# Onetism/LightFieldMicroscopy_PC-bzip2

Measured on AMD Instinct MI355X. Metric: uint16 Mpixel/s encode (predictor->bzip2) at 1/2/4/8 GPUs; ratio parity, higher is better.
Workload: dtype u16

## Files before the change

lightfieldmicroscopy_pc-bzip2_amd/csrc/lfm_bzip2.hip:

```cpp
#include <hip/hip_runtime.h>
#include <rocprim/block/block_exchange.hpp>
#include <rocprim/block/block_sort.hpp>
#include <rocprim/device/device_radix_sort.hpp>
#include <rocprim/device/device_scan.hpp>
#include <rocprim/device/device_segmented_radix_sort.hpp>
#include <rocprim/device/device_select.hpp>
#include <rocprim/iterator/counting_iterator.hpp>
#include <algorithm>
#include <climits>
#include <cstdlib>
#include <cstdint>
#include <cstdio>
#include <cstring>
#include <mutex>
#include <type_traits>
#include <vector>
#include "lfm_bwt_types.h"
#include "lfm_bz_caps.h"
#include "lfm_hip.h"

#ifndef LFM_BWT_FORCE_FULL
#define LFM_BWT_FORCE_FULL 0
#endif

namespace lfm {
namespace bz {

constexpr int kRleThreads = 512;
constexpr int kMaxGroups = 6;
constexpr int kMaxAlpha = 258;
constexpr int kIters = 4;
constexpr uint32_t kRunA = 0, kRunB = 1;

constexpr uint32_t kFlagHost = 1;

struct Geometry {
    uint32_t dims[5];
    uint32_t bs[5];
    uint32_t nb[5];
    uint32_t bpp;
};

struct Batch {
    const uint8_t* img;
    Geometry g;
    uint32_t first_block;
    uint32_t nstreams;
    uint32_t raw_cap;
    uint32_t cap;
    uint32_t level;
    uint32_t nblock_max;
    uint32_t out_cap;
    uint8_t* raw;
    uint32_t* raw_len;
    uint8_t* T;
    uint32_t* n;
    uint32_t* crc;
    uint32_t* inuse;
    uint32_t* flags;
    uint32_t* done;
    uint64_t* keys_a;
    uint64_t* keys_b;
    uint32_t* vals_a;
    uint32_t* sa;
    uint32_t* rank;
    uint32_t* vals_b;
    uint32_t* cl0;
    uint32_t* cl1;
    uint8_t* uflag;
    uint32_t* seg_begin;
    uint32_t* seg_end;
    uint16_t* mtfv;
    uint32_t* nmtf;
    uint32_t* mtf_freq;
    uint32_t* orig_ptr;
    uint8_t* sel;
    uint8_t* sel_mtf;
    uint32_t sel_cap;
    uint32_t* nsel;
    uint32_t* ngroups;
    uint8_t* len;
    uint32_t* code;
    uint32_t* rfreq;
    uint32_t* words;
    uint32_t* out_bytes;
    uint32_t* wide;
    uint32_t* wide_cnt;
    uint32_t* nsub;
    uint32_t* bwt_mode;
    uint32_t* abcnt;
    uint32_t* itab;
    uint2* ent;
    uint32_t it_full;
    uint32_t parts;
    uint32_t full_cap;
    uint8_t* Tfull;
    uint32_t* part_toff;
    uint32_t* part_roff;
    uint32_t* part_rlen;
    uint32_t* out_bits;
    uint32_t* nparts;
    uint32_t* sflags;
    uint32_t* sbytes;
    uint32_t* jwords;
    uint32_t jcap;
    uint32_t pay_cap;
};

__device__ __forceinline__ void block_box(const Geometry& g, uint32_t id, uint32_t org[5], uint32_t sz[5])
{
#pragma unroll
    for (int d = 0; d < 5; ++d) {
        const uint32_t q = id % g.nb[d];
        id /= g.nb[d];
        org[d] = q * g.bs[d];
        sz[d] = min(g.bs[d], g.dims[d] - org[d]);
    }
}

__global__ __launch_bounds__(256) void gather_blocks(Batch B)
{
    const uint32_t s = blockIdx.y;
    uint32_t org[5], sz[5];
    block_box(B.g, B.first_block + s, org, sz);
    const uint32_t rowb = sz[0] * B.g.bpp;
    const uint32_t nrows = sz[1] * sz[2] * sz[3] * sz[4];
    uint8_t* dst = B.raw + (size_t)s * B.raw_cap;
    for (uint32_t r = blockIdx.x; r < nrows; r += gridDim.x) {
        uint32_t q = r;
        const uint32_t y = q % sz[1]; q /= sz[1];
        const uint32_t z = q % sz[2]; q /= sz[2];
        const uint32_t c = q % sz[3]; q /= sz[3];
        const uint32_t t = q;
        const size_t src = ((((size_t)(org[4] + t) * B.g.dims[3] + (org[3] + c)) * B.g.dims[2] + (org[2] + z)) *
                                B.g.dims[1] + (org[1] + y)) * B.g.dims[0] + org[0];
        const uint8_t* sp = B.img + src * B.g.bpp;
        uint8_t* dp = dst + (size_t)r * rowb;
        for (uint32_t i = threadIdx.x; i < rowb; i += blockDim.x) dp[i] = sp[i];
    }
    if (blockIdx.x == 0 && threadIdx.x == 0) B.raw_len[s] = rowb * nrows;
}

struct RunSum {
    uint32_t len;
    uint32_t first, last;
    uint32_t lead;
    uint32_t trail;
};

__device__ __forceinline__ RunSum run_combine(const RunSum& a, const RunSum& b)
{
    const bool ae = a.len == 0, be = b.len == 0;
    const bool join = a.last == b.first && !ae && !be;
    RunSum r;
    r.len = a.len + b.len;
    r.first = ae ? b.first : a.first;
    r.last = be ? a.last : b.last;
    r.lead = ae ? b.lead : ((join && a.lead == a.len) ? a.len + b.lead : a.lead);
    r.trail = be ? a.trail : ((join && b.trail == b.len) ? b.len + a.trail : b.trail);
    return r;
}

__device__ __forceinline__ RunSum run_shfl_up(const RunSum& a, int d)
{
    RunSum r;
    r.len = __shfl_up(a.len, d);
    r.first = __shfl_up(a.first, d);
    r.last = __shfl_up(a.last, d);
    r.lead = __shfl_up(a.lead, d);
    r.trail = __shfl_up(a.trail, d);
    return r;
}
// ... 2236 lines not shown
            tile_out[rle2_swz(wr + w - 1u)] = (uint16_t)EOB;
            atomicAdd(&freq[EOB], 1u);
        }
        __syncthreads();
        const uint32_t base = s_wr;
        for (uint32_t i = t; i < tile_total; i += kRle2Threads) out[base + i] = tile_out[rle2_swz(i)];
        __syncthreads();
        if (t == 0) {
            s_wr = base + tile_total;
            s_carry = tile_end_zeros;
        }
        __syncthreads();
    }
    static_assert(kRunA == 0 && kRunB == 1, "RUNA / RUNB are symbols 0 and 1");
    uint32_t cnts[6] = {nrunA, nrunB, (uint32_t)(hot & 0xFFFFu), (uint32_t)((hot >> 16) & 0xFFFFu),
                        (uint32_t)((hot >> 32) & 0xFFFFu), (uint32_t)(hot >> 48)};
#pragma unroll
    for (int r = 0; r < 6; ++r) {
        uint32_t c = cnts[r];
        for (int d = 32; d > 0; d >>= 1) c += (uint32_t)__shfl_xor((int)c, d);
        if (lane == 0 && c) atomicAdd(&freq[r], c);
    }
    __syncthreads();
    if (t == 0) {
        B.nmtf[s] = s_wr;
        if (!heap_narrow(B, s, (int)nin + 2)) B.wide[atomicAdd(B.wide_cnt, 1u)] = s;
    }
    for (uint32_t v = t; v < kMaxAlpha; v += kRle2Threads) B.mtf_freq[(size_t)s * kMaxAlpha + v] = freq[v];
}

constexpr int kHuffThreads = 256;

__device__ __forceinline__ uint32_t stream_nin(const Batch& B, uint32_t s)
{
    uint32_t nin = 0;
    for (int q = 0; q < 8; ++q) nin += __popc(B.inuse[s * 8 + q]);
    return nin;
}

__global__ __launch_bounds__(64) void huff_init(Batch B)
{
    __shared__ int mf[kMaxAlpha];
    __shared__ int pgs[kMaxGroups], pge[kMaxGroups];
    const uint32_t s = blockIdx.x, t = threadIdx.x;
    if (B.flags[s] & kFlagHost) return;
    const uint32_t nMTF = B.nmtf[s];
    const int alphaSize = (int)stream_nin(B, s) + 2;
    const uint32_t* mfreq = B.mtf_freq + (size_t)s * kMaxAlpha;
    uint8_t* len = B.len + (size_t)s * kMaxGroups * kMaxAlpha;
    const int nGroups = nMTF < 200 ? 2 : nMTF < 600 ? 3 : nMTF < 1200 ? 4 : nMTF < 2400 ? 5 : 6;
    for (int v = t; v < kMaxAlpha; v += 64) mf[v] = v < alphaSize ? (int)mfreq[v] : 0;
    __syncthreads();
    if (t == 0) {
        int nPart = nGroups, remF = (int)nMTF, gs = 0;
        while (nPart > 0) {
            const int tFreq = remF / nPart;
            int ge = gs - 1, aFreq = 0;
            while (aFreq < tFreq && ge < alphaSize - 1) {
                ++ge;
                aFreq += mf[ge];
            }
            if (ge > gs && nPart != nGroups && nPart != 1 && ((nGroups - nPart) % 2 == 1)) {
                aFreq -= mf[ge];
                --ge;
            }
            pgs[nPart - 1] = gs;
            pge[nPart - 1] = ge;
            --nPart;
            gs = ge + 1;
            remF -= aFreq;
        }
        B.ngroups[s] = (uint32_t)nGroups;
        B.nsel[s] = (nMTF + kGSize - 1) / kGSize;
    }
    __syncthreads();
    for (int i = t; i < kMaxGroups * kMaxAlpha; i += 64) {
        const int q = i / kMaxAlpha, v = i - q * kMaxAlpha;
        len[i] = (q < nGroups && v < alphaSize && v >= pgs[q] && v <= pge[q]) ? 0 : 15;
    }
}

__global__ __launch_bounds__(kHuffThreads) void huff_select_reg(Batch B)
{
    __shared__ uint32_t rfreq[kMaxGroups][kMaxAlpha];
    __shared__ uint64_t lpack[kMaxAlpha + 1];
    __shared__ uint32_t junk[kHuffThreads];
    const uint32_t s = blockIdx.x, t = threadIdx.x;
    if (B.flags[s] & kFlagHost) return;
    const uint32_t nMTF = B.nmtf[s], nSel = B.nsel[s];
    const int nGroups = (int)B.ngroups[s];
    const int alphaSize = (int)stream_nin(B, s) + 2;
    const uint8_t* len = B.len + (size_t)s * kMaxGroups * kMaxAlpha;
    const uint16_t* mtfv = B.mtfv + (size_t)s * (B.cap + 8);
    uint8_t* sel = B.sel + (size_t)s * B.sel_cap;
    for (int i = t; i < kMaxGroups * kMaxAlpha; i += kHuffThreads) rfreq[i / kMaxAlpha][i % kMaxAlpha] = 0;
    for (int v = t; v <= kMaxAlpha; v += kHuffThreads) {
        uint64_t lp = 0;
        if (v < alphaSize)
            for (int q = 0; q < nGroups; ++q) lp |= (uint64_t)len[q * kMaxAlpha + v] << (10 * q);
        lpack[v] = lp;
    }
    __syncthreads();
    uint64_t lp_hot[4];
#pragma unroll
    for (int f = 0; f < 4; ++f) lp_hot[f] = lpack[f];
    for (uint32_t g = t; g < nSel; g += kHuffThreads) {
        const uint32_t gs = g * kGSize, cnt = min(nMTF - gs, (uint32_t)kGSize);
        uint32_t w[kGSize / 2];
        if (cnt == (uint32_t)kGSize) {
            const uint32_t* p = (const uint32_t*)(mtfv + gs);
#pragma unroll
            for (int q = 0; q < kGSize / 2; ++q) w[q] = p[q];
        } else {
#pragma unroll
            for (int q = 0; q < kGSize / 2; ++q) {
                const uint32_t lo = 2u * q < cnt ? mtfv[gs + 2 * q] : (uint32_t)kMaxAlpha;
                const uint32_t hi = 2u * q + 1 < cnt ? mtfv[gs + 2 * q + 1] : (uint32_t)kMaxAlpha;
                w[q] = lo | (hi << 16);
            }
        }
        uint32_t hot = 0;
        uint64_t acc = 0;
#pragma unroll
        for (int q = 0; q < kGSize / 2; ++q) {
            const uint32_t lo = w[q] & 0xFFFFu, hi = w[q] >> 16;
            hot += lo < 4u ? 1u << (8u * lo) : 0u;
            hot += hi < 4u ? 1u << (8u * hi) : 0u;
            acc += lpack[lo < 4u ? (uint32_t)kMaxAlpha : lo] + lpack[hi < 4u ? (uint32_t)kMaxAlpha : hi];
        }
#pragma unroll
        for (uint32_t f = 0; f < 4; ++f) acc += (uint64_t)((hot >> (8u * f)) & 0xFFu) * lp_hot[f];
        int bt = -1;
        uint32_t bc = 999999999u;
        for (int q = 0; q < nGroups; ++q) {
            const uint32_t cq = (uint32_t)(acc >> (10 * q)) & 1023u;
            if (cq < bc) { bc = cq; bt = q; }
        }
        sel[g] = (uint8_t)bt;
#pragma unroll
        for (int q = 0; q < kGSize / 2; ++q) {
            const uint32_t lo = w[q] & 0xFFFFu, hi = w[q] >> 16;
            atomicAdd(lo >= 4u && lo != (uint32_t)kMaxAlpha ? &rfreq[bt][lo] : &junk[t], 1u);
            atomicAdd(hi >= 4u && hi != (uint32_t)kMaxAlpha ? &rfreq[bt][hi] : &junk[t], 1u);
        }
#pragma unroll
        for (uint32_t f = 0; f < 4; ++f)
            if ((hot >> (8u * f)) & 0xFFu) atomicAdd(&rfreq[bt][f], (hot >> (8u * f)) & 0xFFu);
    }
    __syncthreads();
    uint32_t* rf = B.rfreq + (size_t)s * kMaxGroups * kMaxAlpha;
    for (int i = t; i < kMaxGroups * kMaxAlpha; i += kHuffThreads) rf[i] = rfreq[i / kMaxAlpha][i % kMaxAlpha];
}

template <typename Ent>
struct HeapQuad {
    Ent e[4];
};

constexpr int kHeapQuads = (kMaxAlpha + 2 + 3) / 4 + 1;

template <typename Ent, int kL>
__device__ __forceinline__ void heap_code_lengths(const Batch& B, char* hb, uint32_t lane, uint32_t s, uint32_t tb)
{
    constexpr int kQuads = kHeapQuads;
    constexpr uint32_t QB = sizeof(HeapQuad<Ent>);
    constexpr uint32_t QS = QB * kL;
    constexpr uint32_t ES = sizeof(Ent);
    const uint32_t lb = lane * QB;
    auto ent = [&](uint32_t e) -> Ent& { return *(Ent*)(hb + (e >> 2) * QS + lb + (e & 3) * ES); };
    {
        const int A = (int)stream_nin(B, s) + 2;
        const uint32_t* freq = B.rfreq + ((size_t)s * kMaxGroups + tb) * kMaxAlpha;
        uint8_t* len = B.len + ((size_t)s * kMaxGroups + tb) * kMaxAlpha;
        uint16_t* parent = (uint16_t*)(B.code + ((size_t)s * kMaxGroups + tb) * kMaxAlpha);
        auto dep = [&](uint32_t k) -> uint16_t& {
            return *(uint16_t*)((char*)&ent(k / (ES / 2)) + 2 * (k % (ES / 2)));
        };
        auto ld2 = [](const void* p, int i) { return *(const uint2*)((const uint32_t*)p + (i > 0 ? i : 0)); };
        constexpr Ent kW = ~(Ent)1023;
        constexpr Ent kSent = ~(Ent)0;
        auto sift = [&](Ent k) {
            const Ent kk = k | (Ent)1023;
            uint32_t zz = 1, ea = lb + ES, ca = lb + 2u * ES;
            Ent cx = ent(2), cy = ent(3), root = k;
            bool go = true, first = true;
            while (true) {
                const uint32_t ga = min(zz, (uint32_t)kQuads - 1u) * QS + lb;
                const HeapQuad<Ent> g = *(const HeapQuad<Ent>*)(hb + ga);
                __builtin_amdgcn_sched_barrier(0);
                const uint32_t r = (cy | (Ent)1023) < cx ? 1u : 0u;
                const Ent ky = r ? cy : cx;
                go = go && !(kk < ky);
                *(Ent*)(hb + ea) = ky;
                if (first) root = go ? ky : k;
                first = false;
                const uint32_t zn = (zz << 1) | r, en = ca + r * ES;
                ca = ga + r * (2u * ES);
                ea = go ? en : ea;
                zz = go ? zn : zz;
                __builtin_amdgcn_sched_barrier(0);
                cx = r ? g.e[2] : g.e[0];
                cy = r ? g.e[3] : g.e[1];
                if (!__builtin_amdgcn_ballot_w64(go)) break;
            }
            *(Ent*)(hb + ea) = k;
            return root;
        };
        auto upheap = [&](uint32_t z, Ent k) {
            bool go = true;
            while (true) {
                const Ent up = ent(z >> 1);
                go = go && k < (up & kW);
                ent(z) = go ? up : k;
                z = go ? z >> 1 : z;
                if (!__any(go)) break;
            }
            return z;
        };
        auto upheap_init = [&](uint32_t z) {
            constexpr int D = 9;
            Ent v[D + 1];
#pragma unroll
            for (int j = 0; j <= D; ++j) v[j] = ent(z >> j);
            __builtin_amdgcn_sched_barrier(0);
            const Ent k = v[0], kk = k | (Ent)1023;
            bool below = true;
#pragma unroll
            for (int j = 0; j < D; ++j) {
                const bool lt = kk < v[j + 1];
                ent(z >> j) = lt ? v[j + 1] : (below || j == 0 ? k : v[j]);
                below = lt;
            }
        };
        int retries = 0, nNodes = A;
        while (true) {
            ent(0) = 0;
            for (int q = (A + 1) >> 2; q < kQuads; ++q) {
#pragma unroll
                for (int j = 0; j < 4; ++j)
                    if (4 * q + j > A) ent((uint32_t)(4 * q + j)) = kSent;
            }
            for (int i0 = 1; i0 <= A; i0 += 32) {
                uint2 f[16];
#pragma unroll
                for (int q = 0; q < 16; ++q) f[q] = ld2(freq, min(i0 - 1 + 2 * q, kMaxAlpha - 2));
#pragma unroll
                for (int q = 0; q < 16; ++q) {
                    const int i = i0 + 2 * q;
                    uint32_t w0 = f[q].x ? f[q].x : 1u, w1 = f[q].y ? f[q].y : 1u;
                    for (int r = 0; r < retries; ++r) {
                        w0 = 1u + w0 / 2u;
                        w1 = 1u + w1 / 2u;
                    }
                    if (i <= A) ent(i) = ((Ent)w0 << 15) | (Ent)i;
                    if (i + 1 <= A) ent(i + 1) = ((Ent)w1 << 15) | (Ent)(i + 1);
                }
            }
            for (int i = 1; i <= A; ++i) upheap_init((uint32_t)i);
            int nHeap = A;
            nNodes = A;
            uint32_t tooLong = 0;
            Ent top = ent(1);
            while (nHeap > 1) {
                const Ent k1 = top;
                const Ent l1 = ent(nHeap);
                ent(nHeap) = kSent;
                --nHeap;
                const Ent k2 = sift(l1);
                const Ent l2 = ent(nHeap);
                ent(nHeap) = kSent;
                --nHeap;
                const Ent r2 = sift(l2);
                ++nNodes;
                parent[(uint32_t)k1 & 1023u] = (uint16_t)nNodes;
                parent[(uint32_t)k2 & 1023u] = (uint16_t)nNodes;
                const uint32_t h1 = (uint32_t)(k1 >> 10) & 31u, h2 = (uint32_t)(k2 >> 10) & 31u;
                const uint32_t h = min(30u, 1u + max(h1, h2));
                tooLong |= h > 17u ? 1u : 0u;
                const Ent kn = ((((k1 >> 15) + (k2 >> 15)) << 5 | (Ent)h) << 10) | (Ent)nNodes;
                ++nHeap;
                top = upheap((uint32_t)nHeap, kn) == 1u ? kn : r2;
            }
            if (!tooLong) break;
            ++retries;
        }
        if (retries) atomicAdd(B.wide_cnt + 1, (uint32_t)retries);
        dep(nNodes) = 0;
        for (int kc = (nNodes - 1) & ~63; kc >= 0; kc -= 64) {
            uint2 pw[16];
#pragma unroll
            for (int q = 0; q < 16; ++q) pw[q] = ld2(parent, min(kc / 2 + 2 * q, (2 * kMaxAlpha) / 2 - 2));
#pragma unroll
            for (int q = 15; q >= 0; --q) {
                const int b = kc + 4 * q;
                const uint32_t p4[4] = {pw[q].x & 0xFFFFu, pw[q].x >> 16, pw[q].y & 0xFFFFu, pw[q].y >> 16};
                uint32_t d[4], dn[4];
#pragma unroll
                for (int r = 0; r < 4; ++r) d[r] = dep(min(p4[r], 2u * kMaxAlpha));
#pragma unroll
                for (int r = 3; r >= 0; --r) {
                    const int k = b + r;
                    uint32_t x = d[r];
#pragma unroll
                    for (int u = r + 1; u < 4; ++u) x = p4[r] == (uint32_t)(b + u) ? dn[u] : x;
                    dn[r] = k == nNodes ? 0u : x + 1u;
                    if (k >= 1 && k < nNodes) dep(k) = (uint16_t)dn[r];
                }
            }
        }
        for (int i = 1; i <= A; ++i) len[i - 1] = (uint8_t)dep(i);
    }
}

template <int kL>
__global__ __launch_bounds__(64) void huff_lengths_heap(Batch B, uint32_t nwg_wide, uint32_t nwide_streams)
{
    __shared__ HeapQuad<uint32_t> hq[kHeapQuads * kL];
    char* hb = (char*)hq;
    const uint32_t lane = threadIdx.x;
    if (blockIdx.x >= nwg_wide) {
        const uint32_t task = (blockIdx.x - nwg_wide) * kL + lane;
        const uint32_t s = task / kMaxGroups, tb = task % kMaxGroups;
        if (lane >= (uint32_t)kL || s >= B.nstreams || (B.flags[s] & kFlagHost) || tb >= B.ngroups[s]) return;
        if (!heap_narrow(B, s, (int)stream_nin(B, s) + 2)) return;
        heap_code_lengths<uint32_t, kL>(B, hb, lane, s, tb);
    } else {
        constexpr int kW = kL / 2;
        const uint32_t i = blockIdx.x * kW + lane;
        if (lane >= (uint32_t)kW || i >= nwide_streams * kMaxGroups) return;
        const uint32_t s = B.wide[i / kMaxGroups], tb = i % kMaxGroups;
        if ((B.flags[s] & kFlagHost) || tb >= B.ngroups[s]) return;
        heap_code_lengths<uint64_t, kW>(B, hb, lane, s, tb);
    }
}

__global__ __launch_bounds__(64) void huff_final(Batch B)
{
    const uint32_t s = blockIdx.x, lane = threadIdx.x;
    if (B.flags[s] & kFlagHost) return;
    const uint32_t nGroups = B.ngroups[s];
    const uint32_t nSel = B.nsel[s];
    const uint32_t alphaSize = stream_nin(B, s) + 2;
    const uint8_t* len = B.len + (size_t)s * kMaxGroups * kMaxAlpha;
    {
        const uint8_t* sel = B.sel + (size_t)s * B.sel_cap;
        uint8_t* sm = B.sel_mtf + (size_t)s * B.sel_cap;
        uint32_t pos = 0x543210u;
        for (uint32_t i0 = 0; i0 < nSel; i0 += 64) {
            const uint32_t cnt = min(64u, nSel - i0);
            const uint32_t v = lane < cnt ? sel[i0 + lane] : 0u;
            uint32_t out = 0;
            for (uint32_t g = 0; g < cnt; ++g) {
                const uint32_t ll = __builtin_amdgcn_readlane(v, g);
                const uint32_t x = pos ^ (ll * 0x111111u);
                const uint32_t z = (x - 0x111111u) & ~x & 0x888888u;
                const uint32_t j = (uint32_t)__builtin_ctz(z) >> 2;
                const uint32_t m = (1u << (4 * (j + 1))) - 1u;
                pos = (pos & ~m) | (((pos << 4) | ll) & m);
                out = lane == g ? j : out;
            }
            if (lane < cnt) sm[i0 + lane] = (uint8_t)out;
        }
    }
    const uint64_t lt = (1ull << lane) - 1ull;
    for (uint32_t q = 0; q < nGroups; ++q) {
        const uint8_t* lq = len + q * kMaxAlpha;
        uint32_t* code = B.code + ((size_t)s * kMaxGroups + q) * kMaxAlpha;
        uint32_t L[5], c[5];
#pragma unroll
        for (int k = 0; k < 5; ++k) {
            const uint32_t i = 64 * k + lane;
            L[k] = i < alphaSize ? lq[i] : 0u;
            c[k] = 0;
        }
        uint32_t vec = 0;
        for (uint32_t nl = 1; nl <= 20; ++nl) {
            uint32_t before = 0;
#pragma unroll
            for (int k = 0; k < 5; ++k) {
                const uint64_t b = __ballot(L[k] == nl);
                if (L[k] == nl) c[k] = vec + before + (uint32_t)__popcll(b & lt);
                before += (uint32_t)__popcll(b);
            }
            vec = (vec + before) << 1;
        }
#pragma unroll
        for (int k = 0; k < 5; ++k) {
            const uint32_t i = 64 * k + lane;
            if (i < alphaSize) code[i] = c[k];
        }
    }
}

constexpr int kEmitThreads = 256;

__device__ __forceinline__ void put_bits_atomic(uint32_t* words, uint64_t pos, uint32_t nbits, uint32_t v)
{
    if (!nbits) return;
    const uint32_t w = (uint32_t)(pos >> 5), o = (uint32_t)(pos & 31);
    const uint64_t sh = ((uint64_t)v << (64 - nbits)) >> o;
    const uint32_t hi = (uint32_t)(sh >> 32), lo = (uint32_t)sh;
    if (hi) atomicOr(&words[w], hi);
    if (lo) atomicOr(&words[w + 1], lo);
}

constexpr uint32_t kSelLds = 8192;

constexpr uint32_t kHdrWords = 4096;

__device__ __forceinline__ void put_bits_hdr(uint32_t* hdr, uint32_t* words, uint64_t pos, uint32_t nbits, uint32_t v)
{
    if (!nbits) return;
    const uint32_t w = (uint32_t)(pos >> 5), o = (uint32_t)(pos & 31);
    const uint64_t sh = ((uint64_t)v << (64 - nbits)) >> o;
    const uint32_t hi = (uint32_t)(sh >> 32), lo = (uint32_t)sh;
    if (w + 1 < kHdrWords) {
        hdr[w] |= hi;
        hdr[w + 1] |= lo;
    } else {
        if (hi) atomicOr(&words[w], hi);
        if (lo) atomicOr(&words[w + 1], lo);
    }
}

__device__ __forceinline__ void put_bits_hdr_atomic(uint32_t* hdr, uint32_t* words, uint64_t pos, uint32_t nbits,
                                                    uint32_t v)
{
    if (!nbits) return;
    const uint32_t w = (uint32_t)(pos >> 5), o = (uint32_t)(pos & 31);
    const uint64_t sh = ((uint64_t)v << (64 - nbits)) >> o;
    const uint32_t hi = (uint32_t)(sh >> 32), lo = (uint32_t)sh;
    if (w + 1 < kHdrWords) {
        if (hi) atomicOr(&hdr[w], hi);
        if (lo) atomicOr(&hdr[w + 1], lo);
    } else {
        if (hi) atomicOr(&words[w], hi);
        if (lo) atomicOr(&words[w + 1], lo);
    }
}

__device__ __forceinline__ void put_bits64_hdr_atomic(uint32_t* hdr, uint32_t* words, uint64_t pos, uint32_t nbits,
                                                      uint64_t v)
{
    if (nbits > 32) {
        put_bits_hdr_atomic(hdr, words, pos, nbits - 32, (uint32_t)(v >> 32));
        put_bits_hdr_atomic(hdr, words, pos + nbits - 32, 32, (uint32_t)v);
    } else {
        put_bits_hdr_atomic(hdr, words, pos, nbits, (uint32_t)v);
    }
}

template <int NT>
__device__ __forceinline__ uint32_t block_excl_scan(uint32_t v, uint32_t* wsum, uint32_t* total)
{
    const uint32_t t = threadIdx.x, lane = t & 63, wave = t >> 6;
    uint32_t inc = v;
#pragma unroll
    for (int d = 1; d < 64; d <<= 1) {
        const uint32_t o = __shfl_up(inc, d);
        if ((int)lane >= d) inc += o;
    }
    if (lane == 63) wsum[wave] = inc;
    __syncthreads();
    uint32_t pre = 0, tot = 0;
#pragma unroll
    for (uint32_t w = 0; w < NT / 64; ++w) {
        const uint32_t x = wsum[w];
        pre += w < wave ? x : 0u;
        tot += x;
    }
// ... 980 lines not shown
```

Before: 18000.

## Rework GPU Huffman heap sift using preference bitmask and fixed-depth unrolled paths

Replaces the data-dependent sift-down loop in the per-lane Huffman heap with a precomputed bitmask of which child is smaller at each node. Each sift can then load its whole root-to-leaf path at once and run a fixed-depth unrolled pass. The depth is chosen per merge step from a wave-uniform heap size, and the retry loop is restructured so all lanes step together. The heap layout changes from quads to a flat per-lane strided array. This aims to cut serial LDS round trips in code-length construction, at the cost of extra bookkeeping to keep the bitmask up to date, more registers, and more complex control flow.

```diff
diff --git a/lightfieldmicroscopy_pc-bzip2_amd/csrc/lfm_bzip2.hip b/lightfieldmicroscopy_pc-bzip2_amd/csrc/lfm_bzip2.hip
--- a/lightfieldmicroscopy_pc-bzip2_amd/csrc/lfm_bzip2.hip
+++ b/lightfieldmicroscopy_pc-bzip2_amd/csrc/lfm_bzip2.hip
@@ -18,6 +18,7 @@
 #include "lfm_bwt_types.h"
 #include "lfm_bz_caps.h"
 #include "lfm_hip.h"
+#include "lfm_huff_heap.h"
 
 #ifndef LFM_BWT_FORCE_FULL
 #define LFM_BWT_FORCE_FULL 0
@@ -2560,71 +2561,48 @@
     for (int i = t; i < kMaxGroups * kMaxAlpha; i += kHuffThreads) rf[i] = rfreq[i / kMaxAlpha][i % kMaxAlpha];
 }
 
+template <typename Ent, int kL>
+struct LdsHeap {
+    static constexpr uint32_t RS = sizeof(Ent) * kL;
+    char* base;
+    uint16_t* parent;
+    __device__ __forceinline__ Ent ld(uint32_t e) const { return *(const Ent*)(base + e * RS); }
+    __device__ __forceinline__ void st(uint32_t e, Ent v) const { *(Ent*)(base + e * RS) = v; }
+    __device__ __forceinline__ void ld_pair(uint32_t e, Ent& a, Ent& b) const
+    {
+        const char* q = base + e * RS;
+        a = *(const Ent*)q;
+        b = *(const Ent*)(q + RS);
+    }
+    __device__ __forceinline__ void fence() const { __builtin_amdgcn_sched_barrier(0); }
+    __device__ __forceinline__ void set_parent(uint32_t node, uint32_t p) const { parent[node] = (uint16_t)p; }
+    __device__ __forceinline__ bool any(bool b) const { return __builtin_amdgcn_ballot_w64(b) != 0; }
+    __device__ __forceinline__ void note_sift(uint32_t, uint32_t) const {}
+    __device__ __forceinline__ void note_push(uint32_t, uint32_t) const {}
+    __device__ __forceinline__ void check(const HeapPref&, uint32_t) const {}
+};
+
 template <typename Ent>
-struct HeapQuad {
-    Ent e[4];
-};
-
-constexpr int kHeapQuads = (kMaxAlpha + 2 + 3) / 4 + 1;
+constexpr int kHeapMaxRetries = sizeof(Ent) == 4 ? 17 : 32;
 
 template <typename Ent, int kL>
 __device__ __forceinline__ void heap_code_lengths(const Batch& B, char* hb, uint32_t lane, uint32_t s, uint32_t tb)
 {
-    constexpr int kQuads = kHeapQuads;
-    constexpr uint32_t QB = sizeof(HeapQuad<Ent>);
-    constexpr uint32_t QS = QB * kL;
     constexpr uint32_t ES = sizeof(Ent);
-    const uint32_t lb = lane * QB;
-    auto ent = [&](uint32_t e) -> Ent& { return *(Ent*)(hb + (e >> 2) * QS + lb + (e & 3) * ES); };
+    static_assert(kHeapEntries * sizeof(Ent) * kL <= 33792, "the heaps' LDS grew");
+    static_assert(kHeapEntries >= kMaxAlpha + 2 && 2 * kMaxAlpha / (int)(ES / 2) < kHeapEntries, "heap entries");
     {
         const int A = (int)stream_nin(B, s) + 2;
         const uint32_t* freq = B.rfreq + ((size_t)s * kMaxGroups + tb) * kMaxAlpha;
         uint8_t* len = B.len + ((size_t)s * kMaxGroups + tb) * kMaxAlpha;
         uint16_t* parent = (uint16_t*)(B.code + ((size_t)s * kMaxGroups + tb) * kMaxAlpha);
+        LdsHeap<Ent, kL> acc{hb + lane * ES, parent};
+        auto ent = [&](uint32_t e) -> Ent& { return *(Ent*)(acc.base + e * LdsHeap<Ent, kL>::RS); };
         auto dep = [&](uint32_t k) -> uint16_t& {
             return *(uint16_t*)((char*)&ent(k / (ES / 2)) + 2 * (k % (ES / 2)));
         };
         auto ld2 = [](const void* p, int i) { return *(const uint2*)((const uint32_t*)p + (i > 0 ? i : 0)); };
-        constexpr Ent kW = ~(Ent)1023;
         constexpr Ent kSent = ~(Ent)0;
-        auto sift = [&](Ent k) {
-            const Ent kk = k | (Ent)1023;
-            uint32_t zz = 1, ea = lb + ES, ca = lb + 2u * ES;
-            Ent cx = ent(2), cy = ent(3), root = k;
-            bool go = true, first = true;
-            while (true) {
-                const uint32_t ga = min(zz, (uint32_t)kQuads - 1u) * QS + lb;
-                const HeapQuad<Ent> g = *(const HeapQuad<Ent>*)(hb + ga);
-                __builtin_amdgcn_sched_barrier(0);
-                const uint32_t r = (cy | (Ent)1023) < cx ? 1u : 0u;
-                const Ent ky = r ? cy : cx;
-                go = go && !(kk < ky);
-                *(Ent*)(hb + ea) = ky;
-                if (first) root = go ? ky : k;
-                first = false;
-                const uint32_t zn = (zz << 1) | r, en = ca + r * ES;
-                ca = ga + r * (2u * ES);
-                ea = go ? en : ea;
-                zz = go ? zn : zz;
-                __builtin_amdgcn_sched_barrier(0);
-                cx = r ? g.e[2] : g.e[0];
-                cy = r ? g.e[3] : g.e[1];
-                if (!__builtin_amdgcn_ballot_w64(go)) break;
-            }
-            *(Ent*)(hb + ea) = k;
-            return root;
-        };
-        auto upheap = [&](uint32_t z, Ent k) {
-            bool go = true;
-            while (true) {
-                const Ent up = ent(z >> 1);
-                go = go && k < (up & kW);
-                ent(z) = go ? up : k;
-                z = go ? z >> 1 : z;
-                if (!__any(go)) break;
-            }
-            return z;
-        };
         auto upheap_init = [&](uint32_t z) {
             constexpr int D = 9;
             Ent v[D + 1];
@@ -2640,58 +2618,51 @@
                 below = lt;
             }
         };
-        int retries = 0, nNodes = A;
-        while (true) {
-            ent(0) = 0;
-            for (int q = (A + 1) >> 2; q < kQuads; ++q) {
-#pragma unroll
-                for (int j = 0; j < 4; ++j)
-                    if (4 * q + j > A) ent((uint32_t)(4 * q + j)) = kSent;
-            }
-            for (int i0 = 1; i0 <= A; i0 += 32) {
-                uint2 f[16];
-#pragma unroll
-                for (int q = 0; q < 16; ++q) f[q] = ld2(freq, min(i0 - 1 + 2 * q, kMaxAlpha - 2));
-#pragma unroll
-                for (int q = 0; q < 16; ++q) {
-                    const int i = i0 + 2 * q;
-                    uint32_t w0 = f[q].x ? f[q].x : 1u, w1 = f[q].y ? f[q].y : 1u;
-                    for (int r = 0; r < retries; ++r) {
-                        w0 = 1u + w0 / 2u;
-                        w1 = 1u + w1 / 2u;
+        int retries = 0;
+        uint32_t nMerged = (uint32_t)A;
+        bool build = true;
+        for (int round = 0; round <= kHeapMaxRetries<Ent>; ++round) {
+            uint32_t nHeap = 1, tooLong = 0;
+            Ent top = 0;
+            HeapPref m;
+            if (build) {
+                ent(0) = 0;
+                for (int e = A + 1; e < kHeapEntries; ++e) ent((uint32_t)e) = kSent;
+                for (int i0 = 1; i0 <= A; i0 += 32) {
+                    uint2 f[16];
+#pragma unroll
+                    for (int q = 0; q < 16; ++q) f[q] = ld2(freq, min(i0 - 1 + 2 * q, kMaxAlpha - 2));
+#pragma unroll
+                    for (int q = 0; q < 16; ++q) {
+                        const int i = i0 + 2 * q;
+                        uint32_t w0 = f[q].x ? f[q].x : 1u, w1 = f[q].y ? f[q].y : 1u;
+                        for (int r = 0; r < retries; ++r) {
+                            w0 = 1u + w0 / 2u;
+                            w1 = 1u + w1 / 2u;
+                        }
+                        if (i <= A) ent(i) = ((Ent)w0 << 15) | (Ent)i;
+                        if (i + 1 <= A) ent(i + 1) = ((Ent)w1 << 15) | (Ent)(i + 1);
                     }
-                    if (i <= A) ent(i) = ((Ent)w0 << 15) | (Ent)i;
-                    if (i + 1 <= A) ent(i + 1) = ((Ent)w1 << 15) | (Ent)(i + 1);
                 }
-            }
-            for (int i = 1; i <= A; ++i) upheap_init((uint32_t)i);
-            int nHeap = A;
-            nNodes = A;
-            uint32_t tooLong = 0;
-            Ent top = ent(1);
-            while (nHeap > 1) {
-                const Ent k1 = top;
-                const Ent l1 = ent(nHeap);
-                ent(nHeap) = kSent;
-                --nHeap;
-                const Ent k2 = sift(l1);
-                const Ent l2 = ent(nHeap);
-                ent(nHeap) = kSent;
-                --nHeap;
-                const Ent r2 = sift(l2);
-                ++nNodes;
-                parent[(uint32_t)k1 & 1023u] = (uint16_t)nNodes;
-                parent[(uint32_t)k2 & 1023u] = (uint16_t)nNodes;
-                const uint32_t h1 = (uint32_t)(k1 >> 10) & 31u, h2 = (uint32_t)(k2 >> 10) & 31u;
-                const uint32_t h = min(30u, 1u + max(h1, h2));
-                tooLong |= h > 17u ? 1u : 0u;
-                const Ent kn = ((((k1 >> 15) + (k2 >> 15)) << 5 | (Ent)h) << 10) | (Ent)nNodes;
-                ++nHeap;
-                top = upheap((uint32_t)nHeap, kn) == 1u ? kn : r2;
-            }
-            if (!tooLong) break;
-            ++retries;
-        }
+                for (int i = 1; i <= A; ++i) upheap_init((uint32_t)i);
+                heap_pref_build<Ent>(acc, m, (uint32_t)A);
+                nHeap = (uint32_t)A;
+                nMerged = (uint32_t)A;
+                top = ent(1);
+            }
+            uint32_t hmax = 0;
+            for (int b = 8; b >= 0; --b) {
+                const uint32_t a = build ? (uint32_t)A : 0u;
+                if (__builtin_amdgcn_ballot_w64((a >> b & 1u) && (a >> (b + 1)) == (hmax >> (b + 1)))) hmax |= 1u << b;
+            }
+            hmax = min(__builtin_amdgcn_readfirstlane(hmax), (uint32_t)kMaxAlpha);
+            for (; hmax > 1u; --hmax)
+                if (build && nHeap > 1u) heap_merge_step_at<Ent>(acc, m, hmax, nHeap, nMerged, top, tooLong);
+            build = build && tooLong && retries < kHeapMaxRetries<Ent>;
+            if (build) ++retries;
+            if (!__builtin_amdgcn_ballot_w64(build)) break;
+        }
+        const int nNodes = (int)nMerged;
         if (retries) atomicAdd(B.wide_cnt + 1, (uint32_t)retries);
         dep(nNodes) = 0;
         for (int kc = (nNodes - 1) & ~63; kc >= 0; kc -= 64) {
@@ -2723,7 +2694,7 @@
 template <int kL>
 __global__ __launch_bounds__(64) void huff_lengths_heap(Batch B, uint32_t nwg_wide, uint32_t nwide_streams)
 {
-    __shared__ HeapQuad<uint32_t> hq[kHeapQuads * kL];
+    __shared__ uint32_t hq[kHeapEntries * kL];
     char* hb = (char*)hq;
     const uint32_t lane = threadIdx.x;
     if (blockIdx.x >= nwg_wide) {
diff --git a/lightfieldmicroscopy_pc-bzip2_amd/csrc/lfm_huff_heap.h b/lightfieldmicroscopy_pc-bzip2_amd/csrc/lfm_huff_heap.h
--- /dev/null
+++ b/lightfieldmicroscopy_pc-bzip2_amd/csrc/lfm_huff_heap.h
@@ -0,0 +1,256 @@
+#pragma once
+#include <cstdint>
+
+#ifndef LFM_HD
+#if defined(__HIPCC__) || defined(__CUDACC__)
+#define LFM_HD __host__ __device__
+#else
+#define LFM_HD
+#endif
+#endif
+
+constexpr int kHeapEntries = 264;
+constexpr uint32_t kHeapSentPair = 260;
+constexpr int kHeapMaxLevels = 8;
+constexpr int kPrefWords = 5;
+
+struct HeapPref {
+    uint32_t w[kPrefWords];
+};
+
+template <typename Ent>
+LFM_HD inline bool heap_wless(Ent a, Ent b)
+{
+    return (a | (Ent)1023) < b;
+}
+
+template <typename Ent>
+LFM_HD inline Ent heap_sent()
+{
+    return ~(Ent)0;
+}
+
+LFM_HD inline uint32_t heap_pref_at(const HeapPref& m, int j, uint32_t p)
+{
+    if (j <= 4) return (m.w[0] >> (p & 31u)) & 1u;
+    if (j == 5) return (m.w[1] >> (p & 31u)) & 1u;
+    if (j == 6) return ((p & 32u ? m.w[3] : m.w[2]) >> (p & 31u)) & 1u;
+    const uint32_t b = p - 128u < 31u ? p - 128u : 31u;
+    return (m.w[4] >> b) & 1u;
+}
+
+LFM_HD inline uint32_t heap_put_bit(uint32_t w, uint32_t b, uint32_t bit)
+{
+    return (w & ~(1u << b)) | (bit << b);
+}
+
+LFM_HD inline void heap_pref_flip(HeapPref& d, int j, uint32_t p, uint32_t flip)
+{
+    if (j <= 4) {
+        d.w[0] |= flip << (p & 31u);
+    } else if (j == 5) {
+        d.w[1] |= flip << (p & 31u);
+    } else if (j == 6) {
+        const uint32_t x = flip << (p & 31u);
+        d.w[2] |= p & 32u ? 0u : x;
+        d.w[3] |= p & 32u ? x : 0u;
+    } else {
+        const uint32_t b = p - 128u < 31u ? p - 128u : 31u;
+        d.w[4] |= flip << b;
+    }
+}
+
+LFM_HD inline void heap_pref_set_any(HeapPref& m, uint32_t p, uint32_t bit)
+{
+    const uint32_t b = p & 31u, wi = p >> 5;
+#pragma unroll
+    for (uint32_t i = 0; i < (uint32_t)kPrefWords; ++i) m.w[i] = wi == i ? heap_put_bit(m.w[i], b, bit) : m.w[i];
+}
+
+template <typename Ent, typename Acc>
+LFM_HD inline void heap_pref_build(Acc& acc, HeapPref& m, uint32_t A)
+{
+    const uint32_t last = A >> 1;
+#pragma unroll
+    for (uint32_t wi = 0; wi < (uint32_t)kPrefWords; ++wi) {
+        uint32_t word = 0;
+        for (uint32_t b0 = 0; b0 < 32u && 32u * wi + b0 <= last; b0 += 8u) {
+            Ent l[8], r[8];
+#pragma unroll
+            for (uint32_t q = 0; q < 8u; ++q) {
+                const uint32_t p = 32u * wi + b0 + q;
+                acc.ld_pair(2u * (p <= last ? p : last), l[q], r[q]);
+            }
+            acc.fence();
+#pragma unroll
+            for (uint32_t q = 0; q < 8u; ++q) {
+                const uint32_t p = 32u * wi + b0 + q;
+                word |= (p >= 1u && p <= last && heap_wless(r[q], l[q]) ? 1u : 0u) << (b0 + q);
+            }
+        }
+        m.w[wi] = word;
+    }
+}
+
+template <int L, typename Ent, typename Acc>
+LFM_HD inline Ent heap_sift_path(Acc& acc, HeapPref& m, Ent k)
+{
+    if constexpr (L == 0) {
+        acc.st(1u, k);
+        acc.note_sift(0u, 0u);
+        return k;
+    } else {
+        uint32_t p[L + 1], cb[L], r[L];
+        p[0] = 1u;
+#pragma unroll
+        for (int j = 0; j < L; ++j) {
+            r[j] = heap_pref_at(m, j, p[j]);
+            cb[j] = 2u * p[j];
+            if (j == 7) cb[j] = cb[j] < kHeapSentPair ? cb[j] : kHeapSentPair;
+            p[j + 1] = cb[j] | r[j];
+        }
+        Ent a[L], b[L];
+#pragma unroll
+        for (int j = 0; j < L; ++j) acc.ld_pair(cb[j], a[j], b[j]);
+        acc.fence();
+        const Ent kk = k | (Ent)1023;
+        Ent c[L], sib[L], nv[L + 1];
+        bool go[L];
+        bool g = true;
+        uint32_t went = 0;
+#pragma unroll
+        for (int j = 0; j < L; ++j) {
+            c[j] = r[j] ? b[j] : a[j];
+            sib[j] = r[j] ? a[j] : b[j];
+            g = g && !(kk < c[j]);
+            go[j] = g;
+            went += g ? 1u : 0u;
+        }
+        nv[0] = go[0] ? c[0] : k;
+#pragma unroll
+        for (int j = 1; j < L; ++j) nv[j] = go[j] ? c[j] : (go[j - 1] ? k : c[j - 1]);
+        nv[L] = go[L - 1] ? k : c[L - 1];
+#pragma unroll
+        for (int j = 0; j <= L; ++j) acc.st(p[j], nv[j]);
+        HeapPref d = {{0u, 0u, 0u, 0u, 0u}};
+#pragma unroll
+        for (int j = 0; j < L; ++j) {
+            const Ent right = r[j] ? nv[j + 1] : sib[j], left = r[j] ? sib[j] : nv[j + 1];
+            heap_pref_flip(d, j, p[j], r[j] ^ (heap_wless(right, left) ? 1u : 0u));
+        }
+#pragma unroll
+        for (int i = 0; i < kPrefWords; ++i) m.w[i] ^= d.w[i];
+        acc.note_sift(went, (uint32_t)L);
+        return nv[0];
+    }
+}
+
+template <typename Ent, typename Acc>
+LFM_HD inline Ent heap_pop_last(Acc& acc, HeapPref& m, uint32_t& nHeap)
+{
+    const Ent last = acc.ld(nHeap);
+    acc.st(nHeap, heap_sent<Ent>());
+    heap_pref_set_any(m, nHeap >> 1, 0u);
+    --nHeap;
+    return last;
+}
+
+constexpr int kPushAhead = 3;
+
+template <typename Ent, typename Acc>
+LFM_HD inline uint32_t heap_push(Acc& acc, HeapPref& m, uint32_t z, Ent k)
+{
+    constexpr Ent kW = ~(Ent)1023;
+    const uint32_t from = z;
+    Ent upa[kPushAhead], sba[kPushAhead];
+#pragma unroll
+    for (int t = 0; t < kPushAhead; ++t) {
+        upa[t] = acc.ld(z >> (t + 1));
+        sba[t] = acc.ld((z >> t) ^ 1u);
+    }
+    acc.fence();
+    bool go = true;
+    Ent up = upa[0], sib = sba[0];
+    auto step = [&]() {
+        go = go && k < (up & kW);
+        const Ent v = go ? up : k;
+        acc.st(z, v);
+        if (z >= 2u) {
+            const Ent right = z & 1u ? v : sib, left = z & 1u ? sib : v;
+            heap_pref_set_any(m, z >> 1, heap_wless(right, left) ? 1u : 0u);
+        }
+        z = go ? z >> 1 : z;
+        return acc.any(go);
+    };
+    bool more = step();
+#pragma unroll
+    for (int t = 1; t < kPushAhead; ++t) {
+        if (!more) break;
+        up = go ? upa[t] : up;
+        sib = go ? sba[t] : sib;
+        more = step();
+    }
+    for (int t = kPushAhead; more && t < kHeapMaxLevels + 1; ++t) {
+        up = acc.ld(z >> 1);
+        sib = acc.ld(z ^ 1u);
+        more = step();
+    }
+    acc.note_push(from, z);
+    return z;
+}
+
+template <int L, typename Ent, typename Acc>
+LFM_HD inline void heap_merge_step(Acc& acc, HeapPref& m, uint32_t& nHeap, uint32_t& nNodes, Ent& top, uint32_t& tooLong)
+{
+    const Ent k1 = top;
+    const Ent l1 = heap_pop_last<Ent>(acc, m, nHeap);
+    acc.check(m, nHeap);
+    const Ent k2 = heap_sift_path<L, Ent>(acc, m, l1);
+    acc.check(m, nHeap);
+    const Ent l2 = heap_pop_last<Ent>(acc, m, nHeap);
+    acc.check(m, nHeap);
+    const Ent r2 = heap_sift_path<L, Ent>(acc, m, l2);
+    acc.check(m, nHeap);
+    ++nNodes;
+    acc.set_parent((uint32_t)k1 & 1023u, nNodes);
+    acc.set_parent((uint32_t)k2 & 1023u, nNodes);
+    const uint32_t h1 = (uint32_t)(k1 >> 10) & 31u, h2 = (uint32_t)(k2 >> 10) & 31u;
+    const uint32_t hm = h1 > h2 ? h1 : h2;
+    const uint32_t h = hm + 1u < 30u ? hm + 1u : 30u;
+    tooLong |= h > 17u ? 1u : 0u;
+    const Ent kn = ((((k1 >> 15) + (k2 >> 15)) << 5 | (Ent)h) << 10) | (Ent)nNodes;
+    ++nHeap;
+    top = heap_push<Ent>(acc, m, nHeap, kn) == 1u ? kn : r2;
+    acc.check(m, nHeap);
+}
+
+LFM_HD inline int heap_levels(uint32_t n)
+{
+    return 31 - __builtin_clz(n);
+}
+
+template <typename Ent, typename Acc>
+LFM_HD inline void heap_merge_step_at(Acc& acc, HeapPref& m, uint32_t hmax, uint32_t& nHeap, uint32_t& nNodes, Ent& top,
+                                      uint32_t& tooLong)
+{
+    switch (heap_levels(hmax - 1u)) {
+    case 0: heap_merge_step<0, Ent>(acc, m, nHeap, nNodes, top, tooLong); break;
+    case 1: heap_merge_step<1, Ent>(acc, m, nHeap, nNodes, top, tooLong); break;
+    case 2: heap_merge_step<2, Ent>(acc, m, nHeap, nNodes, top, tooLong); break;
+    case 3: heap_merge_step<3, Ent>(acc, m, nHeap, nNodes, top, tooLong); break;
+    case 4: heap_merge_step<4, Ent>(acc, m, nHeap, nNodes, top, tooLong); break;
+    case 5: heap_merge_step<5, Ent>(acc, m, nHeap, nNodes, top, tooLong); break;
+    case 6: heap_merge_step<6, Ent>(acc, m, nHeap, nNodes, top, tooLong); break;
+    case 7: heap_merge_step<7, Ent>(acc, m, nHeap, nNodes, top, tooLong); break;
+    default: heap_merge_step<8, Ent>(acc, m, nHeap, nNodes, top, tooLong); break;
+    }
+}
+
+template <typename Ent, typename Acc>
+LFM_HD inline void heap_merge_all(Acc& acc, HeapPref& m, uint32_t A, uint32_t hmax, uint32_t& nNodes, uint32_t& tooLong)
+{
+    uint32_t nHeap = A;
+    Ent top = acc.ld(1u);
+    for (uint32_t it = 0; it + 1u < hmax; ++it)
+        if (nHeap > 1u) heap_merge_step_at<Ent>(acc, m, hmax - it, nHeap, nNodes, top, tooLong);
+}
```

New measurement: 18190 (median of 6 runs). 1.01x the previous value.
